# THU-LYJ-Lab/AR-Seg

Measured on AMD Instinct MI355X. Metric: non-keyframe frames/sec (backbone+CReFF) at 512x1024, higher is better.
Workload: dtype f32

## Files before the change

### ar-seg_amd/csrc/conv_up2_c64.hip

```cpp
#include "arseg_device.h"
#include "conv_plans.h"
#include <cmath>

namespace {

constexpr int TH = 8, TW = 16, PH = TH + 2, PW = TW + 2, NPX = PH * PW;
constexpr int PLANE = NPX * 64, BUFB = 4 * PLANE;
constexpr int BWC = PW / 2, NBLK = (PH / 2) * BWC;
constexpr int NMMA = 256, NSTAGE = 256, NT = NMMA + NSTAGE;
constexpr int MAXU = (NBLK * 16 + NSTAGE - 1) / NSTAGE;
constexpr int KT = 18;
constexpr unsigned OOB = 0x80000000u;
enum { ROLE_MMA = 0, ROLE_STAGE = 1 };

struct Up2Params {
    const float *in, *w, *scale, *bias;
    float *out;
    int H, W, in_ld, out_ld;
    int tiles_x, tiles_y, ntiles;
    int act;
    float slope;
    unsigned *range_flag;
    float range_limit;
    unsigned in_bytes, w_bytes, out_bytes;
};

struct TileRun { int first, stride, count; };
__device__ __forceinline__ TileRun tile_run(int ntiles) {
    const int G = (int)gridDim.x, b = (int)blockIdx.x, nx = G < 8 ? G : 8;
    const int xcd = b % nx, idx = b / nx, wgs = (G - xcd + nx - 1) / nx;
    const int q = ntiles / nx, r = ntiles - q * nx;
    const int start = xcd < r ? xcd * (q + 1) : r * (q + 1) + (xcd - r) * q, cnt = q + (xcd < r ? 1 : 0);
    return TileRun{start + idx, wgs, idx < cnt ? (cnt - idx + wgs - 1) / wgs : 0};
}
struct TilePos { int img, ty0, tx0; };
__device__ __forceinline__ TilePos tile_pos(const Up2Params &p, int t) {
    const int per = p.tiles_x * p.tiles_y, img = t / per, rem = t - img * per, ty = rem / p.tiles_x;
    return TilePos{img, ty * TH, (rem - ty * p.tiles_x) * TW};
}

template <int ROLE>
__device__ __forceinline__ void up2_role(const Up2Params &p, unsigned char *lds) {
    const TileRun run = tile_run(p.ntiles);
    if (run.count == 0) return;

    if constexpr (ROLE == ROLE_STAGE) {
        const int ptid = (int)threadIdx.x - NMMA;
        const __amdgpu_buffer_rsrc_t a_rsrc = __builtin_amdgcn_make_buffer_rsrc(const_cast<float *>(p.in), 0, (int)p.in_bytes, 0x00020000);
        const bool watch = p.range_flag != nullptr;
        float vmax = 0.f;
        const int h = p.H >> 1, w = p.W >> 1;
        int by[MAXU], bx[MAXU], upx[MAXU];
#pragma unroll
        for (int it = 0; it < MAXU; ++it) {
            const int b = (ptid + it * NSTAGE) >> 4;
            by[it] = b / BWC; bx[it] = b - by[it] * BWC;
            upx[it] = b < NBLK ? 2 * by[it] * PW + 2 * bx[it] : -1;
        }
        const int p16 = ptid & 15;
        u32x4 rq[MAXU][4];
        int uflag[MAXU];
        auto load_quads = [&](int t) {
            const TilePos tp = tile_pos(p, t);
#pragma unroll
            for (int it = 0; it < MAXU; ++it) {
                const int iy = (tp.ty0 >> 1) - 1 + by[it], ix = (tp.tx0 >> 1) - 1 + bx[it];
                const int ya = min(max(iy, 0), h - 1), yb = min(max(iy + 1, 0), h - 1), xa = min(max(ix, 0), w - 1), xb = min(max(ix + 1, 0), w - 1);
                const unsigned base = (unsigned)(tp.img * h) * (unsigned)w, q16 = (unsigned)p16 * 16u;
                const bool live = upx[it] >= 0;
                const unsigned o0 = live ? ((base + ya * w + xa) * p.in_ld) * 4u + q16 : OOB, o1 = live ? ((base + ya * w + xb) * p.in_ld) * 4u + q16 : OOB;
                const unsigned o2 = live ? ((base + yb * w + xa) * p.in_ld) * 4u + q16 : OOB, o3 = live ? ((base + yb * w + xb) * p.in_ld) * 4u + q16 : OOB;
                rq[it][0] = __builtin_amdgcn_raw_buffer_load_b128(a_rsrc, o0, 0, 0);
                rq[it][1] = __builtin_amdgcn_raw_buffer_load_b128(a_rsrc, o1, 0, 0);
                rq[it][2] = __builtin_amdgcn_raw_buffer_load_b128(a_rsrc, o2, 0, 0);
                rq[it][3] = __builtin_amdgcn_raw_buffer_load_b128(a_rsrc, o3, 0, 0);
                uflag[it] = ((iy >= 0 && 2 * iy + 1 < p.H) ? 1 : 0) | ((2 * iy + 2 < p.H) ? 2 : 0) | ((ix >= 0 && 2 * ix + 1 < p.W) ? 4 : 0) |
                            ((2 * ix + 2 < p.W) ? 8 : 0) | (iy < 0 ? 16 : 0) | (ix < 0 ? 32 : 0);
            }
        };
        auto stage = [&](unsigned char *buf) {
            auto put_px = [&](int px, const f32x4 v) {
                u32x2 hi, lo;
                split4(v, hi, lo);
                if (watch) vmax = fmaxf(fmaxf(vmax, fmaxf(fabsf(v[0]), fabsf(v[1]))), fmaxf(fabsf(v[2]), fabsf(v[3])));
                const int piece = p16 & 7;
                unsigned char *row = buf + (p16 >> 3) * 2 * PLANE + px * 64 + (((piece >> 1) ^ ((px >> 1) & 2)) << 4) + (piece & 1) * 8;
                *reinterpret_cast<u32x2 *>(row) = hi;
                *reinterpret_cast<u32x2 *>(row + PLANE) = lo;
            };
#pragma unroll
            for (int it = 0; it < MAXU; ++it) {
                if (upx[it] < 0) continue;
                const int f = uflag[it];
                const f32x4 q00 = __builtin_bit_cast(f32x4, rq[it][0]), q01 = __builtin_bit_cast(f32x4, rq[it][1]);
                const f32x4 q10 = __builtin_bit_cast(f32x4, rq[it][2]), q11 = __builtin_bit_cast(f32x4, rq[it][3]);
                const f32x4 r0a = 0.75f * q00 + 0.25f * q10, r0b = 0.75f * q01 + 0.25f * q11;
                const f32x4 r1a = (f & 16) ? q10 : 0.25f * q00 + 0.75f * q10, r1b = (f & 16) ? q11 : 0.25f * q01 + 0.75f * q11;
                const f32x4 z = {0.f, 0.f, 0.f, 0.f};
                const f32x4 o00 = 0.75f * r0a + 0.25f * r0b, o01 = (f & 32) ? r0b : 0.25f * r0a + 0.75f * r0b;
                const f32x4 o10 = 0.75f * r1a + 0.25f * r1b, o11 = (f & 32) ? r1b : 0.25f * r1a + 0.75f * r1b;
                put_px(upx[it], (f & 5) == 5 ? o00 : z);
                put_px(upx[it] + 1, (f & 9) == 9 ? o01 : z);
                put_px(upx[it] + PW, (f & 6) == 6 ? o10 : z);
                put_px(upx[it] + PW + 1, (f & 10) == 10 ? o11 : z);
            }
        };
        load_quads(run.first);
#pragma unroll 1
        for (int j = -1; j < run.count; ++j) {
            if (j + 1 < run.count) {
                stage(lds + ((j + 1) & 1) * BUFB);
                if (j + 2 < run.count) load_quads(run.first + (j + 2) * run.stride);
            }
            __syncthreads();
        }
        if (watch && vmax > p.range_limit) atomicOr(p.range_flag, 1u);
    } else {
        const int lane = (int)threadIdx.x & 63, slice = (int)threadIdx.x >> 6, l15 = lane & 15, kg = lane >> 4;
        h16x8 wh[KT], wl[KT];
        {
            const __amdgpu_buffer_rsrc_t b_rsrc = __builtin_amdgcn_make_buffer_rsrc(const_cast<float *>(p.w), 0, (int)p.w_bytes, 0x00020000);
            const unsigned wo = (unsigned)((slice * 16 + l15) * KT) * 128u + (unsigned)kg * 16u;
#pragma unroll
            for (int kt = 0; kt < KT; ++kt) {
                wh[kt] = __builtin_bit_cast(h16x8, __builtin_amdgcn_raw_buffer_load_b128(b_rsrc, wo + kt * 128, 0, 0));
                wl[kt] = __builtin_bit_cast(h16x8, __builtin_amdgcn_raw_buffer_load_b128(b_rsrc, wo + kt * 128 + 64, 0, 0));
            }
        }
        const int c0 = slice * 16 + kg * 4;
        float sc[4], bi[4];
#pragma unroll
        for (int r = 0; r < 4; ++r) { sc[r] = p.scale ? p.scale[c0 + r] : 1.0f; bi[r] = p.bias ? p.bias[c0 + r] : 0.0f; }
        const ArsegAct ea = arseg_act(p.act, p.slope);
        const u32x4 o_rsrc = make_rsrc(p.out, p.out_bytes);
        unsigned swz[8];
#pragma unroll
        for (int j = 0; j < 8; ++j) swz[j] = (unsigned)(l15 * 64 + ((kg ^ (((l15 + j) >> 1) & 2)) << 4));

        __syncthreads();
#pragma unroll 1
        for (int j = 0; j < run.count; ++j) {
            const unsigned char *buf = lds + (j & 1) * BUFB;
            const unsigned char *pj[8];
#pragma unroll
            for (int i = 0; i < 8; ++i) pj[i] = buf + swz[i];
            f32x4 acc[TH];
#pragma unroll
            for (int mf = 0; mf < TH; ++mf) acc[mf] = f32x4{0.f, 0.f, 0.f, 0.f};
            h16x8 fh[2][2], fl[2][2];
            auto frags = [&](int g, h16x8 (&h)[2], h16x8 (&l)[2]) {
                const int ck = g / 36, tap = (g % 36) >> 2;
#pragma unroll
                for (int u = 0; u < 2; ++u) {
                    const int C = (2 * (g & 3) + u + tap / 3) * PW + tap % 3;
                    h[u] = *reinterpret_cast<const h16x8 *>(pj[C & 7] + 2 * ck * PLANE + C * 64);
                    l[u] = *reinterpret_cast<const h16x8 *>(pj[C & 7] + (2 * ck + 1) * PLANE + C * 64);
                }
            };
            frags(0, fh[0], fl[0]);
#pragma unroll
            for (int g = 0; g < 72; ++g) {
                if (g + 1 < 72) frags(g + 1, fh[(g + 1) & 1], fl[(g + 1) & 1]);
                const int kt = 2 * ((g % 36) >> 2) + g / 36;
#pragma unroll
                for (int u = 0; u < 2; ++u) {
                    const int mf = 2 * (g & 3) + u;
                    acc[mf] = __builtin_amdgcn_mfma_f32_16x16x32_f16(wh[kt], fl[g & 1][u], acc[mf], 0, 0, 0);
                    acc[mf] = __builtin_amdgcn_mfma_f32_16x16x32_f16(wl[kt], fh[g & 1][u], acc[mf], 0, 0, 0);
                    acc[mf] = __builtin_amdgcn_mfma_f32_16x16x32_f16(wh[kt], fh[g & 1][u], acc[mf], 0, 0, 0);
                }
                __builtin_amdgcn_sched_group_barrier(0x100, 4, 0);
                __builtin_amdgcn_sched_group_barrier(0x008, 6, 0);
                __builtin_amdgcn_sched_barrier(0);
            }
            const TilePos tp = tile_pos(p, run.first + j * run.stride);
            const int ox = tp.tx0 + l15;
#pragma unroll
            for (int mf = 0; mf < TH; ++mf) {
                const int oy = tp.ty0 + mf;
                f32x4 v;
#pragma unroll
                for (int r = 0; r < 4; ++r) v[r] = arseg_act_apply(acc[mf][r] * sc[r] + bi[r], ea);
                const unsigned m = ((unsigned)tp.img * (unsigned)p.H + (unsigned)oy) * (unsigned)p.W + (unsigned)ox;
                store16_buf(__builtin_bit_cast(u32x4, v), o_rsrc, (oy < p.H && ox < p.W) ? (m * (unsigned)p.out_ld + (unsigned)c0) * 4u : OOB);
            }
            __syncthreads();
        }
    }
}

__global__ __launch_bounds__(NT) void conv_up2_c64_kernel(const Up2Params p) {
    extern __shared__ __attribute__((aligned(16))) unsigned char up2_smem[];
    if (threadIdx.x < NMMA) up2_role<ROLE_MMA>(p, up2_smem);
    else up2_role<ROLE_STAGE>(p, up2_smem);
}

}

extern "C" int arseg_conv_up2_c64_fwd(const arseg_conv_desc *d, const float *in, const float *w_packed, const float *scale, const float *bias, float *out,
                                      int max_wgs, arseg_stream_t stream) {
    if (!d) return ARSEG_EINVAL;
    if (d->N <= 0 || d->H <= 0 || d->W <= 0 || max_wgs < 0) return ARSEG_EINVAL;
    if (!conv_up2_c64_shape(d)) return ARSEG_EUNSUPPORTED;
    if (d->in_ld < 64 || (d->in_ld & 3) || d->out_ld < 64) return ARSEG_EINVAL;
    if (d->out_ld & 3) return ARSEG_EUNSUPPORTED;
    if (d->act != ARSEG_ACT_NONE && d->act != ARSEG_ACT_RELU && d->act != ARSEG_ACT_PRELU && d->act != ARSEG_ACT_SIGMOID) return ARSEG_EINVAL;
    ARSEG_CHECK_PTR(in); ARSEG_CHECK_PTR(w_packed); ARSEG_CHECK_PTR(out);
    if (!ARSEG_ALIGNED16(in) || !ARSEG_ALIGNED16(w_packed)) return ARSEG_EINVAL;
    if (!ARSEG_ALIGNED16(out)) return ARSEG_EUNSUPPORTED;
    void *rf = d->range_flag;
    if (rf && (reinterpret_cast<uintptr_t>(rf) & 3)) return ARSEG_EINVAL;
    const long long ib = conv_up2_c64_in_bytes(d), ob = conv_up2_c64_out_bytes(d);
    if ((long long)d->N * d->H * d->W > (1ll << 30) || ib >= (1ll << 31) || ob >= (1ll << 31)) return ARSEG_EUNSUPPORTED;
    Up2Params p;
    p.in = in; p.w = w_packed; p.scale = scale; p.bias = bias; p.out = out;
    p.H = d->H; p.W = d->W; p.in_ld = d->in_ld; p.out_ld = d->out_ld;
    p.tiles_x = arseg_cdiv(d->W, TW); p.tiles_y = arseg_cdiv(d->H, TH); p.ntiles = d->N * p.tiles_x * p.tiles_y;
    p.act = d->act; p.slope = d->prelu_slope;
    p.range_flag = reinterpret_cast<unsigned *>(rf);
    p.range_limit = d->range_limit > 0.0f ? d->range_limit : 65504.0f;
    p.in_bytes = (unsigned)ib; p.w_bytes = (unsigned)(64 * KT * 128); p.out_bytes = (unsigned)ob;
    hipStream_t hs = arseg_stream(stream);
    static ArsegSmemAttr attr;
    if (int e = arseg_allow_smem(attr, reinterpret_cast<const void *>(conv_up2_c64_kernel), 2 * BUFB)) return e;
    const int cus = arseg_cu_count(max_wgs), grid = p.ntiles < cus ? p.ntiles : cus;
    hipLaunchKernelGGL(conv_up2_c64_kernel, dim3(grid), dim3(NT), 2 * BUFB, hs, p);
    return arseg_launch_status();
}
```

Baseline: 2384.

## Reorder up2 conv MMA loop by row pairs and pipeline staging loads

The MMA role now accumulates two output rows at a time over all taps and stores each pair right away, instead of keeping eight accumulators for the whole tile and storing at the end. This shortens accumulator live ranges and spreads stores through the tile. The staging role copies prefetched quads into working registers before issuing the next tile's loads, so the loads overlap the LDS staging. __syncthreads is replaced with a raw s_barrier that waits only on lgkmcnt, and the sigmoid branch becomes a compile-time specialization. The extra rn registers and inline-asm moves raise register pressure, and the weaker barrier depends on the vmcnt ordering being correct.

```diff
diff --git a/ar-seg_amd/csrc/conv_up2_c64.hip b/ar-seg_amd/csrc/conv_up2_c64.hip
--- a/ar-seg_amd/csrc/conv_up2_c64.hip
+++ b/ar-seg_amd/csrc/conv_up2_c64.hip
@@ -1,6 +1,7 @@
 #include "arseg_device.h"
 #include "conv_plans.h"
 #include <cmath>
+#include <type_traits>
 
 namespace {
 
@@ -39,6 +40,14 @@
     return TilePos{img, ty * TH, (rem - ty * p.tiles_x) * TW};
 }
 
+__device__ __forceinline__ void tile_barrier() {
+    asm volatile("s_waitcnt lgkmcnt(0)" ::: "memory");
+    __builtin_amdgcn_sched_barrier(0);
+    __builtin_amdgcn_s_barrier();
+    __builtin_amdgcn_sched_barrier(0);
+    asm volatile("" ::: "memory");
+}
+
 template <int ROLE>
 __device__ __forceinline__ void up2_role(const Up2Params &p, unsigned char *lds) {
     const TileRun run = tile_run(p.ntiles);
@@ -58,8 +67,8 @@
             upx[it] = b < NBLK ? 2 * by[it] * PW + 2 * bx[it] : -1;
         }
         const int p16 = ptid & 15;
-        u32x4 rq[MAXU][4];
-        int uflag[MAXU];
+        u32x4 rq[MAXU][4], rn[MAXU][4];
+        int uflag[MAXU], nflag[MAXU];
         auto load_quads = [&](int t) {
             const TilePos tp = tile_pos(p, t);
 #pragma unroll
@@ -70,11 +79,11 @@
                 const bool live = upx[it] >= 0;
                 const unsigned o0 = live ? ((base + ya * w + xa) * p.in_ld) * 4u + q16 : OOB, o1 = live ? ((base + ya * w + xb) * p.in_ld) * 4u + q16 : OOB;
                 const unsigned o2 = live ? ((base + yb * w + xa) * p.in_ld) * 4u + q16 : OOB, o3 = live ? ((base + yb * w + xb) * p.in_ld) * 4u + q16 : OOB;
-                rq[it][0] = __builtin_amdgcn_raw_buffer_load_b128(a_rsrc, o0, 0, 0);
-                rq[it][1] = __builtin_amdgcn_raw_buffer_load_b128(a_rsrc, o1, 0, 0);
-                rq[it][2] = __builtin_amdgcn_raw_buffer_load_b128(a_rsrc, o2, 0, 0);
-                rq[it][3] = __builtin_amdgcn_raw_buffer_load_b128(a_rsrc, o3, 0, 0);
-                uflag[it] = ((iy >= 0 && 2 * iy + 1 < p.H) ? 1 : 0) | ((2 * iy + 2 < p.H) ? 2 : 0) | ((ix >= 0 && 2 * ix + 1 < p.W) ? 4 : 0) |
+                rn[it][0] = __builtin_amdgcn_raw_buffer_load_b128(a_rsrc, o0, 0, 0);
+                rn[it][1] = __builtin_amdgcn_raw_buffer_load_b128(a_rsrc, o1, 0, 0);
+                rn[it][2] = __builtin_amdgcn_raw_buffer_load_b128(a_rsrc, o2, 0, 0);
+                rn[it][3] = __builtin_amdgcn_raw_buffer_load_b128(a_rsrc, o3, 0, 0);
+                nflag[it] = ((iy >= 0 && 2 * iy + 1 < p.H) ? 1 : 0) | ((2 * iy + 2 < p.H) ? 2 : 0) | ((ix >= 0 && 2 * ix + 1 < p.W) ? 4 : 0) |
                             ((2 * ix + 2 < p.W) ? 8 : 0) | (iy < 0 ? 16 : 0) | (ix < 0 ? 32 : 0);
             }
         };
@@ -105,14 +114,29 @@
                 put_px(upx[it] + PW + 1, (f & 10) == 10 ? o11 : z);
             }
         };
+        auto take = [&]() {
+#pragma unroll
+            for (int it = 0; it < MAXU; ++it) {
+#pragma unroll
+                for (int q = 0; q < 4; ++q) {
+                    const u32x2 s01 = {rn[it][q][0], rn[it][q][1]}, s23 = {rn[it][q][2], rn[it][q][3]};
+                    u32x2 d01, d23;
+                    asm volatile("v_mov_b64 %0, %2\n\tv_mov_b64 %1, %3" : "=&v"(d01), "=&v"(d23) : "v"(s01), "v"(s23));
+                    rq[it][q] = u32x4{d01[0], d01[1], d23[0], d23[1]};
+                }
+                asm volatile("v_mov_b32 %0, %1" : "=v"(uflag[it]) : "v"(nflag[it]));
+            }
+        };
         load_quads(run.first);
 #pragma unroll 1
         for (int j = -1; j < run.count; ++j) {
             if (j + 1 < run.count) {
+                take();
+                if (j + 2 < run.count) load_quads(run.first + (j + 2) * run.stride);
+                __builtin_amdgcn_sched_barrier(0);
                 stage(lds + ((j + 1) & 1) * BUFB);
-                if (j + 2 < run.count) load_quads(run.first + (j + 2) * run.stride);
-            }
-            __syncthreads();
+            }
+            tile_barrier();
         }
         if (watch && vmax > p.range_limit) atomicOr(p.range_flag, 1u);
     } else {
@@ -126,66 +150,76 @@
                 wh[kt] = __builtin_bit_cast(h16x8, __builtin_amdgcn_raw_buffer_load_b128(b_rsrc, wo + kt * 128, 0, 0));
                 wl[kt] = __builtin_bit_cast(h16x8, __builtin_amdgcn_raw_buffer_load_b128(b_rsrc, wo + kt * 128 + 64, 0, 0));
             }
+#pragma unroll
+            for (int kt = 0; kt < KT; ++kt) asm volatile("" ::"v"(wh[kt]), "v"(wl[kt]));
         }
         const int c0 = slice * 16 + kg * 4;
         float sc[4], bi[4];
 #pragma unroll
         for (int r = 0; r < 4; ++r) { sc[r] = p.scale ? p.scale[c0 + r] : 1.0f; bi[r] = p.bias ? p.bias[c0 + r] : 0.0f; }
+#pragma unroll
+        for (int r = 0; r < 4; ++r) asm volatile("" ::"v"(sc[r]), "v"(bi[r]));
         const ArsegAct ea = arseg_act(p.act, p.slope);
         const u32x4 o_rsrc = make_rsrc(p.out, p.out_bytes);
         unsigned swz[8];
 #pragma unroll
         for (int j = 0; j < 8; ++j) swz[j] = (unsigned)(l15 * 64 + ((kg ^ (((l15 + j) >> 1) & 2)) << 4));
 
-        __syncthreads();
+        tile_barrier();
+        auto tiles = [&](auto SIG) {
+            const ArsegAct et{ea.slope, ea.relu, decltype(SIG)::value};
 #pragma unroll 1
-        for (int j = 0; j < run.count; ++j) {
-            const unsigned char *buf = lds + (j & 1) * BUFB;
-            const unsigned char *pj[8];
-#pragma unroll
-            for (int i = 0; i < 8; ++i) pj[i] = buf + swz[i];
-            f32x4 acc[TH];
-#pragma unroll
-            for (int mf = 0; mf < TH; ++mf) acc[mf] = f32x4{0.f, 0.f, 0.f, 0.f};
-            h16x8 fh[2][2], fl[2][2];
-            auto frags = [&](int g, h16x8 (&h)[2], h16x8 (&l)[2]) {
-                const int ck = g / 36, tap = (g % 36) >> 2;
-#pragma unroll
-                for (int u = 0; u < 2; ++u) {
-                    const int C = (2 * (g & 3) + u + tap / 3) * PW + tap % 3;
-                    h[u] = *reinterpret_cast<const h16x8 *>(pj[C & 7] + 2 * ck * PLANE + C * 64);
-                    l[u] = *reinterpret_cast<const h16x8 *>(pj[C & 7] + (2 * ck + 1) * PLANE + C * 64);
+            for (int j = 0; j < run.count; ++j) {
+                const unsigned char *buf = lds + (j & 1) * BUFB;
+                const unsigned char *pj[8];
+#pragma unroll
+                for (int i = 0; i < 8; ++i) pj[i] = buf + swz[i];
+                const TilePos tp = tile_pos(p, run.first + j * run.stride);
+                const int ox = tp.tx0 + l15;
+                h16x8 fh[2][2], fl[2][2];
+                auto frags = [&](int G, h16x8 (&h)[2], h16x8 (&l)[2]) {
+                    const int rp = G / 18, ck = (G % 18) / 9, tap = G % 9;
+#pragma unroll
+                    for (int u = 0; u < 2; ++u) {
+                        const int C = (2 * rp + u + tap / 3) * PW + tap % 3;
+                        h[u] = *reinterpret_cast<const h16x8 *>(pj[C & 7] + 2 * ck * PLANE + C * 64);
+                        l[u] = *reinterpret_cast<const h16x8 *>(pj[C & 7] + (2 * ck + 1) * PLANE + C * 64);
+                    }
+                };
+                frags(0, fh[0], fl[0]);
+#pragma unroll
+                for (int rp = 0; rp < TH / 2; ++rp) {
+                    f32x4 acc[2] = {f32x4{0.f, 0.f, 0.f, 0.f}, f32x4{0.f, 0.f, 0.f, 0.f}};
+#pragma unroll
+                    for (int s = 0; s < 18; ++s) {
+                        const int G = rp * 18 + s, kt = 2 * (s % 9) + s / 9;
+                        if (G + 1 < 72) frags(G + 1, fh[(G + 1) & 1], fl[(G + 1) & 1]);
+#pragma unroll
+                        for (int u = 0; u < 2; ++u) {
+                            acc[u] = __builtin_amdgcn_mfma_f32_16x16x32_f16(wh[kt], fl[G & 1][u], acc[u], 0, 0, 0);
+                            acc[u] = __builtin_amdgcn_mfma_f32_16x16x32_f16(wl[kt], fh[G & 1][u], acc[u], 0, 0, 0);
+                            acc[u] = __builtin_amdgcn_mfma_f32_16x16x32_f16(wh[kt], fh[G & 1][u], acc[u], 0, 0, 0);
+                        }
+                        __builtin_amdgcn_sched_group_barrier(0x100, 4, 0);
+                        __builtin_amdgcn_sched_group_barrier(0x008, 6, 0);
+                        __builtin_amdgcn_sched_barrier(0);
+                    }
+#pragma unroll
+                    for (int u = 0; u < 2; ++u) {
+                        const int oy = tp.ty0 + 2 * rp + u;
+                        f32x4 v;
+#pragma unroll
+                        for (int r = 0; r < 4; ++r) v[r] = arseg_act_apply(acc[u][r] * sc[r] + bi[r], et);
+                        const unsigned m = ((unsigned)tp.img * (unsigned)p.H + (unsigned)oy) * (unsigned)p.W + (unsigned)ox;
+                        store16_buf(__builtin_bit_cast(u32x4, v), o_rsrc, (oy < p.H && ox < p.W) ? (m * (unsigned)p.out_ld + (unsigned)c0) * 4u : OOB);
+                    }
+                    __builtin_amdgcn_sched_barrier(0);
                 }
-            };
-            frags(0, fh[0], fl[0]);
-#pragma unroll
-            for (int g = 0; g < 72; ++g) {
-                if (g + 1 < 72) frags(g + 1, fh[(g + 1) & 1], fl[(g + 1) & 1]);
-                const int kt = 2 * ((g % 36) >> 2) + g / 36;
-#pragma unroll
-                for (int u = 0; u < 2; ++u) {
-                    const int mf = 2 * (g & 3) + u;
-                    acc[mf] = __builtin_amdgcn_mfma_f32_16x16x32_f16(wh[kt], fl[g & 1][u], acc[mf], 0, 0, 0);
-                    acc[mf] = __builtin_amdgcn_mfma_f32_16x16x32_f16(wl[kt], fh[g & 1][u], acc[mf], 0, 0, 0);
-                    acc[mf] = __builtin_amdgcn_mfma_f32_16x16x32_f16(wh[kt], fh[g & 1][u], acc[mf], 0, 0, 0);
-                }
-                __builtin_amdgcn_sched_group_barrier(0x100, 4, 0);
-                __builtin_amdgcn_sched_group_barrier(0x008, 6, 0);
-                __builtin_amdgcn_sched_barrier(0);
-            }
-            const TilePos tp = tile_pos(p, run.first + j * run.stride);
-            const int ox = tp.tx0 + l15;
-#pragma unroll
-            for (int mf = 0; mf < TH; ++mf) {
-                const int oy = tp.ty0 + mf;
-                f32x4 v;
-#pragma unroll
-                for (int r = 0; r < 4; ++r) v[r] = arseg_act_apply(acc[mf][r] * sc[r] + bi[r], ea);
-                const unsigned m = ((unsigned)tp.img * (unsigned)p.H + (unsigned)oy) * (unsigned)p.W + (unsigned)ox;
-                store16_buf(__builtin_bit_cast(u32x4, v), o_rsrc, (oy < p.H && ox < p.W) ? (m * (unsigned)p.out_ld + (unsigned)c0) * 4u : OOB);
-            }
-            __syncthreads();
-        }
+                tile_barrier();
+            }
+        };
+        if (ea.sigmoid) tiles(std::true_type{});
+        else tiles(std::false_type{});
     }
 }
 
```

Result: no change. 2390 (median of 4 runs) (+0.2%).
